# rubengooj/stvo-pl

Hardware: AMD Instinct MI355X
Metric: stereo frames/s (match+optimizePose) (higher is better)
Workload: dtype u8/fp4+f64; 1 GPU; BASELINE configs[2]: KITTI-00-shaped stereo with points + lines (ORB + LBD rows), grid-windowed stereo match (points and lines) + f2f brute-force mutual-NNR match (points and lines) + full GN optimizePose (config_kitti.yaml), device-resident per-frame pipeline; the streams cycle through the 8 sequence ids / 3 KITTI calibrations of configs[4] (sequence s on rank s mod G); streams_per_gpu=3072, parallelism=seq-shard x1

## Files before the change

### stvo-pl_amd/csrc/match_mfma.hip

```cpp
#include <type_traits>

#include "kernels.h"

namespace stvo {

typedef int v4i __attribute__((ext_vector_type(4)));
typedef int v8i __attribute__((ext_vector_type(8)));
typedef int v16i __attribute__((ext_vector_type(16)));
typedef float v16f __attribute__((ext_vector_type(16)));

#ifndef MF_TPB
#define MF_TPB 2
#endif
#ifndef MF_FOLD_SLOTS
#define MF_FOLD_SLOTS 5
#endif
constexpr int MF_BLOCK = 256;
constexpr int MF_TILE = 32;
constexpr int MF_KEY_SHIFT = 13;
constexpr int MF_KEY_BIAS = 1 << 20;
constexpr int MF_NO_KEY = 0x7FFFFFFF;
constexpr int MF_NO_KEY_MIN = 0x40000000;

__device__ __forceinline__ v4i expand_fp4(uint32_t w) {
    v4i r;
    r.x = (int)(((w << 3) & 0x88888888u) | 0x66666666u);
    r.y = (int)(((w << 2) & 0x88888888u) | 0x66666666u);
    r.z = (int)(((w << 1) & 0x88888888u) | 0x66666666u);
    r.w = (int)((w & 0x88888888u) | 0x66666666u);
    return r;
}
__device__ __forceinline__ float med3_f32(float a, float b, float c) {
    float r;
    asm("v_med3_f32 %0, %1, %2, %3" : "=v"(r) : "v"(a), "v"(b), "v"(c));
    return r;
}
__device__ __forceinline__ float min_f32(float a, float b) {
    float r;
    asm("v_min_f32 %0, %1, %2" : "=v"(r) : "v"(a), "v"(b));
    return r;
}
__device__ __forceinline__ float max_f32(float a, float b) {
    float r;
    asm("v_max_f32 %0, %1, %2" : "=v"(r) : "v"(a), "v"(b));
    return r;
}
__device__ __forceinline__ float min3_f32(float a, float b, float c) {
    float r;
    asm("v_min3_f32 %0, %1, %2, %3" : "=v"(r) : "v"(a), "v"(b), "v"(c));
    return r;
}
constexpr float MF_NO_KEY_F = 1.0e30f;
constexpr float MF_NO_KEY_MIN_F = 1.0e29f;
constexpr int MF_SCALE_2_4 = 127 + 4;

__device__ __forceinline__ uint32_t key_to_knn(int key, int base) {
    if (key >= MF_NO_KEY_MIN) return 0xFFFFFFFFu;
    const uint32_t u = (uint32_t)(key + base + MF_KEY_BIAS);
    return ((u >> MF_KEY_SHIFT) << 16) | (u & ((1u << MF_KEY_SHIFT) - 1u));
}

template <int QB, int MODE>
__global__ __launch_bounds__(MF_BLOCK, (QB == 1 ? 4 : QB == 2 ? 3 : 1)) void hamming_knn2_mfma_kernel(int B, int tiles, int ndir, int dir0, int nseg, int row_stride,
                                                                      const uint8_t* __restrict__ d1,
                                                                      const int32_t* __restrict__ n1,
                                                                      const uint8_t* __restrict__ d2,
                                                                      const int32_t* __restrict__ n2,
                                                                      uint2* __restrict__ knn12, uint2* __restrict__ knn21,
                                                                      const int32_t* __restrict__ qsel,
                                                                      const int32_t* __restrict__ nsel,
                                                                      uint32_t* __restrict__ claim_init, int qsel_from_back,
                                                                      const int32_t* __restrict__ tsel,
                                                                      const int32_t* __restrict__ ntsel) {
    constexpr bool GATHER = MODE >= 1, TGATHER = MODE == 2;
    constexpr int ROWS = 4 * QB * 32;
    constexpr int KSTEPS = 4;
    using key_t = float;
    using acc_t = v16f;
    constexpr int NBUF = 2 * MF_TPB;
    __shared__ v4i s_tile[NBUF][KSTEPS * 2 * 32];
    const int per_frame = tiles * ndir * nseg;
    const int L = blockIdx.x;
    const int xcd = L & 7, k = L >> 3;
    int fb = k / per_frame, local = k % per_frame;
    if (MODE == 0 && ndir == 1 && tiles > 1) {
        const int groups = (int)(gridDim.x >> 3) / per_frame;
        const int full_pf = (tiles - 1) * nseg, full = full_pf * groups;
        if (k < full) {
            fb = k / full_pf;
            local = k % full_pf;
        } else {
            fb = (k - full) / nseg;
            local = full_pf + (k - full) % nseg;
        }
    }
    const int b = fb * 8 + xcd;
    if (b >= B) return;
    const int seg = local % nseg;
    const int dir = dir0 + (local / nseg) / tiles;
    const int tile = (local / nseg) % tiles;
    const size_t frame_off = (size_t)b * row_stride;
    const int tid = threadIdx.x, lane = tid & 63, wv = tid >> 6, col = lane & 31, hf = lane >> 5;
    const int q_base = tile * ROWS;
    const uint32_t* __restrict__ Q = reinterpret_cast<const uint32_t*>((dir == 0 ? d1 : d2) + frame_off * STVO_DESC_BYTES);
    uint4 qw[QB][2];
    if (!GATHER) {
#pragma unroll
        for (int qb = 0; qb < QB; ++qb) {
            const int qi = min(q_base + (wv * QB + qb) * 32 + col, row_stride - 1);
            qw[qb][0] = reinterpret_cast<const uint4*>(Q)[2 * qi];
            qw[qb][1] = reinterpret_cast<const uint4*>(Q)[2 * qi + 1];
        }
    }
    const int na = n1[b], nb = n2[b];
    const int nq = GATHER ? nsel[b] : (dir == 0 ? na : nb);
    const int nt_all = TGATHER ? ntsel[b] : (dir == 0 ? nb : na);
    if (TGATHER && nt_all == 0) return;
    const int seg_len = (((nt_all + nseg - 1) / nseg) + MF_TILE - 1) & ~(MF_TILE - 1);
    const int j0 = min(seg * seg_len, nt_all);
    const int nt = min(j0 + seg_len, nt_all);
    if (claim_init && seg == 0 && dir == dir0)
        for (int c = q_base + tid; c < min(q_base + ROWS, row_stride); c += MF_BLOCK) claim_init[frame_off + c] = 0xFFFFFFFFu;
    if (q_base >= nq) return;
    const uint32_t* __restrict__ T = reinterpret_cast<const uint32_t*>((dir == 0 ? d2 : d1) + frame_off * STVO_DESC_BYTES);
    uint2* __restrict__ out = (dir == 0 ? knn12 : knn21) + (size_t)seg * B * row_stride + frame_off;

    const bool wave_active = q_base + wv * QB * 32 < nq;
    v4i qf[QB][KSTEPS];
    auto query_row = [&](int qb) {
        const int q = q_base + (wv * QB + qb) * 32 + col;
        const int qc = q < nq ? q : nq - 1;
        return GATHER ? qsel[frame_off + (qsel_from_back ? row_stride - 1 - qc : qc)] : qc;
    };
    if (GATHER) {
#pragma unroll
        for (int qb = 0; qb < QB; ++qb) {
            const int qi = query_row(qb);
            qw[qb][0] = reinterpret_cast<const uint4*>(Q)[2 * qi];
            qw[qb][1] = reinterpret_cast<const uint4*>(Q)[2 * qi + 1];
        }
    }
#pragma unroll
    for (int qb = 0; qb < QB; ++qb) {
        const uint32_t w[8] = {qw[qb][0].x, qw[qb][0].y, qw[qb][0].z, qw[qb][0].w, qw[qb][1].x, qw[qb][1].y, qw[qb][1].z, qw[qb][1].w};
        const bool up = hf != 0;
        qf[qb][0] = expand_fp4(~(up ? w[1] : w[0]));
        qf[qb][1] = expand_fp4(~(up ? w[3] : w[2]));
        qf[qb][2] = expand_fp4(~(up ? w[5] : w[4]));
        qf[qb][3] = expand_fp4(~(up ? w[7] : w[6]));
    }
    acc_t cidx;
#pragma unroll
    for (int r = 0; r < 16; ++r) cidx[r] = (key_t)((r & 3) + 8 * (r >> 2) + 4 * hf);

    const key_t no_key = MF_NO_KEY_F;
    key_t best[QB], second[QB];
#pragma unroll
    for (int qb = 0; qb < QB; ++qb) best[qb] = second[qb] = no_key;

    const int xr = tid & 31, xk = tid >> 5;
    const int ntiles = (nt - j0 + MF_TILE - 1) / MF_TILE;
    auto fetch = [&](int t) -> uint32_t {
        const int j = j0 + t * MF_TILE + xr;
        if (j >= nt) return 0u;
        const int row = TGATHER ? tsel[frame_off + j] : j;
        return T[(size_t)row * 8 + xk];
    };
    auto stage = [&](int t, uint32_t w) {
        s_tile[t & (NBUF - 1)][xk * 32 + xr] = expand_fp4(w);
    };
#pragma unroll
    for (int i = 0; i < MF_TPB; ++i)
        if (i < ntiles) stage(i, fetch(i));
    __syncthreads();
    auto rebase = [&]() {
#pragma unroll
        for (int qb = 0; qb < QB; ++qb) {
            best[qb] -= (key_t)MF_TILE;
            second[qb] -= (key_t)MF_TILE;
        }
    };
    auto fold = [&](int qb, key_t key) {
        second[qb] = med3_f32(best[qb], second[qb], key);
        best[qb] = min_f32(best[qb], key);
    };
    auto mma = [&](const v4i& tf, const v4i& q, const acc_t& c) -> acc_t {
        const v8i a8 = {tf.x, tf.y, tf.z, tf.w, 0, 0, 0, 0}, b8 = {q.x, q.y, q.z, q.w, 0, 0, 0, 0};
        return __builtin_amdgcn_mfma_scale_f32_32x32x64_f8f6f4(a8, b8, c, 4, 4, 0, MF_SCALE_2_4, 0, MF_SCALE_2_4);
    };
    auto mma_fold = [&](acc_t (&cur)[QB], acc_t (&prev)[QB], int t) {
        if (wave_active) {
            const v4i* frag = s_tile[t & (NBUF - 1)];
            const bool fold_prev = t > 0;
            if (fold_prev) rebase();
            key_t node[QB][5];
            v4i tf = frag[lane];
#pragma unroll
            for (int kk = 0; kk < KSTEPS; ++kk) {
                v4i tf_ahead = tf;
                if (kk < KSTEPS - 1) tf_ahead = frag[(kk + 1) * 64 + lane];
#pragma unroll
                for (int qb = 0; qb < QB; ++qb) cur[qb] = mma(tf, qf[qb][kk], kk == 0 ? cidx : cur[qb]);
                if (fold_prev) {
                    if (QB == 1 && kk == 0) asm volatile("s_nop 7\n\ts_nop 7\n\ts_nop 2" : "+v"(prev[0]));
#pragma unroll
                    for (int qb = 0; qb < QB; ++qb) {
                        const acc_t& p = prev[qb];
                        key_t(&a)[5] = node[qb];
                        if (kk == 0) {
                            a[0] = min3_f32(p[0], p[1], p[2]);
                            a[1] = min3_f32(p[3], p[4], p[5]);
                            second[qb] = min3_f32(second[qb], med3_f32(p[0], p[1], p[2]), med3_f32(p[3], p[4], p[5]));
                        } else if (kk == 1) {
                            a[2] = min3_f32(p[6], p[7], p[8]);
                            a[3] = min3_f32(p[9], p[10], p[11]);
                            second[qb] = min3_f32(second[qb], med3_f32(p[6], p[7], p[8]), med3_f32(p[9], p[10], p[11]));
                        } else if (kk == 2) {
                            a[4] = min3_f32(p[12], p[13], p[14]);
                            const key_t b0 = min3_f32(a[0], a[1], a[2]);
                            second[qb] = min3_f32(second[qb], med3_f32(p[12], p[13], p[14]), med3_f32(a[0], a[1], a[2]));
                            a[0] = b0;
                        } else {
                            const key_t b1 = min3_f32(a[3], a[4], p[15]), n1 = med3_f32(a[3], a[4], p[15]);
                            second[qb] = min3_f32(second[qb], n1, med3_f32(a[0], b1, best[qb]));
                            best[qb] = min3_f32(a[0], b1, best[qb]);
                        }
                    }
                }
                if (kk < KSTEPS - 1) __builtin_amdgcn_sched_group_barrier(0x100, 1, 0);
#pragma unroll
                for (int qb = 0; qb < QB; ++qb) {
                    __builtin_amdgcn_sched_group_barrier(0x008, 1, 0);
                    __builtin_amdgcn_sched_group_barrier(0x002, MF_FOLD_SLOTS, 0);
                }
                tf = tf_ahead;
            }
        }
    };
    acc_t accA[QB], accB[QB];
#pragma unroll
    for (int qb = 0; qb < QB; ++qb)
#pragma unroll
        for (int r = 0; r < 16; ++r) accA[qb][r] = accB[qb][r] = 0;
    static_assert(MF_TPB % 2 == 0, "the accumulator sets alternate tile by tile");
    int t = 0;
    uint32_t w_near[MF_TPB];
#pragma unroll
    for (int i = 0; i < MF_TPB; ++i) {
        w_near[i] = 0;
        if (MF_TPB + i < ntiles) w_near[i] = fetch(MF_TPB + i);
    }
    for (; t + MF_TPB <= ntiles; t += MF_TPB) {
        uint32_t w_far[MF_TPB];
#pragma unroll
        for (int i = 0; i < MF_TPB; ++i) {
            w_far[i] = 0;
            if (t + 2 * MF_TPB + i < ntiles) w_far[i] = fetch(t + 2 * MF_TPB + i);
        }
#pragma unroll
        for (int i = 0; i < MF_TPB; ++i) {
            if ((i & 1) == 0) mma_fold(accA, accB, t + i);
            else mma_fold(accB, accA, t + i);
        }
#pragma unroll
        for (int i = 0; i < MF_TPB; ++i) {
            if (t + MF_TPB + i < ntiles) stage(t + MF_TPB + i, w_near[i]);
            w_near[i] = w_far[i];
        }
        __syncthreads();
    }
#pragma unroll
    for (int i = 0; i < MF_TPB - 1; ++i)
        if (t + i < ntiles) {
            if ((i & 1) == 0) mma_fold(accA, accB, t + i);
            else mma_fold(accB, accA, t + i);
        }
    if (wave_active && ntiles > 0) {
        const int jt = j0 + (ntiles - 1) * MF_TILE;
        const acc_t(&last)[QB] = (ntiles & 1) ? accA : accB;
        rebase();
#pragma unroll
        for (int qb = 0; qb < QB; ++qb)
#pragma unroll
            for (int r = 0; r < 16; ++r) {
                const int jr = jt + (r & 3) + 8 * (r >> 2) + 4 * hf;
                fold(qb, jr < nt ? last[qb][r] : no_key);
            }
    }
    if (!wave_active) return;
#pragma unroll
    for (int qb = 0; qb < QB; ++qb) {
        const int bi = best[qb] >= MF_NO_KEY_MIN_F ? MF_NO_KEY : (int)best[qb];
        const int si = second[qb] >= MF_NO_KEY_MIN_F ? MF_NO_KEY : (int)second[qb];
        const int ob = __shfl_xor(bi, 32), os = __shfl_xor(si, 32);
        const int hi = max(bi, ob);
        const int sec = min(min(si, os), hi);
        const int bst = min(bi, ob);
        const int q = q_base + (wv * QB + qb) * 32 + col;
        const int base = j0 + (ntiles - 1) * MF_TILE;
        if (hf == 0 && q < nq) out[query_row(qb)] = make_uint2(key_to_knn(bst, base), key_to_knn(sec, base));
    }
}

constexpr int REV_CHUNK_TILES = 8, REV_CHUNK = REV_CHUNK_TILES * MF_TILE;

__global__ __launch_bounds__(MF_BLOCK, 4) void hamming_knn2_mfma_reverse_kernel(int B, int slots, int row_stride, const uint8_t* __restrict__ d1,
                                                                                const int32_t* __restrict__ n1, const uint8_t* __restrict__ d2,
                                                                                const int32_t* __restrict__ qsel, const int32_t* __restrict__ nsel,
                                                                                const int32_t* __restrict__ tsel, const uint32_t* __restrict__ claim,
                                                                                float nnr, int32_t* __restrict__ m12) {
    constexpr int KSTEPS = 4;
    using key_t = float;
    using acc_t = v16f;
    __shared__ v4i s_tile[REV_CHUNK_TILES][KSTEPS * 2 * 32];
    __shared__ uint16_t s_thr[257];
    const int L = blockIdx.x;
    const int xcd = L & 7, k = L >> 3;
    const int b = (k / slots) * 8 + xcd, slot = k % slots;
    if (b >= B) return;
    const int na = n1[b];
    const int nl = nsel[(size_t)B + b], nh = nsel[2 * (size_t)B + b], ns = nsel[3 * (size_t)B + b];
    if ((ns == 0 || nl == 0) && nh == 0) return;
    {
        const float f0 = (float)threadIdx.x;
        uint32_t thr = threadIdx.x;
        while (thr < 256u && !(f0 < (float)(thr + 1u) * nnr)) ++thr;
        s_thr[threadIdx.x] = (uint16_t)thr;
        if (threadIdx.x == 0) s_thr[256] = 256;
    }
    const size_t frame_off = (size_t)b * row_stride;
    const int tid = threadIdx.x, lane = tid & 63, wv = tid >> 6, col = lane & 31, hf = lane >> 5;
    const int xr = tid & 31, xk = tid >> 5;
    const uint32_t* __restrict__ Q = reinterpret_cast<const uint32_t*>(d2 + frame_off * STVO_DESC_BYTES);
    const uint32_t* __restrict__ T = reinterpret_cast<const uint32_t*>(d1 + frame_off * STVO_DESC_BYTES);
    acc_t cidx;
#pragma unroll
    for (int r = 0; r < 16; ++r) cidx[r] = (key_t)((r & 3) + 8 * (r >> 2) + 4 * hf);
    auto mma = [&](const v4i& tf, const v4i& q, const acc_t& c) -> acc_t {
        const v8i a8 = {tf.x, tf.y, tf.z, tf.w, 0, 0, 0, 0}, b8 = {q.x, q.y, q.z, q.w, 0, 0, 0, 0};
        return __builtin_amdgcn_mfma_scale_f32_32x32x64_f8f6f4(a8, b8, c, 4, 4, 0, MF_SCALE_2_4, 0, MF_SCALE_2_4);
    };

    for (int list = 0; list < 2; ++list) {
        const bool light = list == 0;
        const int nq = light ? (ns > 0 ? nl : 0) : nh, nt_all = light ? ns : na;
        if (nq == 0) continue;
        const int nseg = rev_segments(nt_all);
        const int n_groups = (nq + 127) / 128;
        const int seg_len = (((nt_all + nseg - 1) / nseg) + MF_TILE - 1) & ~(MF_TILE - 1);
        auto column_of = [&](int g) -> int {
            const int q = (g * 4 + wv) * 32 + col;
            return q < nq ? q : nq - 1;
        };
        auto list_entry = [&](int g) -> int { return qsel[frame_off + (light ? column_of(g) : row_stride - 1 - column_of(g))]; };
        for (int seg = 0; seg < nseg; ++seg) {
            const int g_first = ((slot - seg) % slots + slots) % slots;
            if (g_first >= n_groups) continue;
            const int j0 = min(seg * seg_len, nt_all), nt = min(j0 + seg_len, nt_all);
            for (int c0 = j0; c0 < nt || c0 == j0; c0 += REV_CHUNK) {
                uint32_t w[REV_CHUNK_TILES];
#pragma unroll
                for (int t = 0; t < REV_CHUNK_TILES; ++t) {
                    const int j = c0 + t * MF_TILE + xr;
                    uint32_t v = 0u;
                    if (j < nt) v = T[(size_t)(light ? tsel[frame_off + j] : j) * 8 + xk];
                    w[t] = v;
                }
                int e_cur = list_entry(g_first);
                int e_next = g_first + slots < n_groups ? list_entry(g_first + slots) : 0;
                const int ntc = min((nt - c0 + MF_TILE - 1) / MF_TILE, REV_CHUNK_TILES);
#pragma unroll
                for (int t = 0; t < REV_CHUNK_TILES; ++t)
                    if (t < ntc) s_tile[t][xk * 32 + xr] = expand_fp4(w[t]);
                uint4 qw0 = reinterpret_cast<const uint4*>(Q)[2 * e_cur], qw1 = reinterpret_cast<const uint4*>(Q)[2 * e_cur + 1];
                uint32_t cw = claim[frame_off + e_cur];
                __syncthreads();
                for (int g = g_first; g < n_groups; g += slots) {
                    const bool up = hf != 0;
                    v4i qf[KSTEPS];
                    qf[0] = expand_fp4(~(up ? qw0.y : qw0.x));
                    qf[1] = expand_fp4(~(up ? qw0.w : qw0.z));
                    qf[2] = expand_fp4(~(up ? qw1.y : qw1.x));
                    qf[3] = expand_fp4(~(up ? qw1.w : qw1.z));
                    const uint32_t c_claim = cw;
                    const bool block_active = (g * 4 + wv) * 32 < nq;
                    if (g + slots < n_groups) {
                        qw0 = reinterpret_cast<const uint4*>(Q)[2 * e_next];
                        qw1 = reinterpret_cast<const uint4*>(Q)[2 * e_next + 1];
                        cw = claim[frame_off + e_next];
                        e_cur = e_next;
                        if (g + 2 * slots < n_groups) e_next = list_entry(g + 2 * slots);
                    }
                    if (!block_active) continue;
                    key_t best = MF_NO_KEY_F, second = MF_NO_KEY_F;
                    auto fold = [&](key_t key) {
                        second = med3_f32(best, second, key);
                        best = min_f32(best, key);
                    };
                    int last_base = c0;
                    if (ntc > 0) {
                        auto do_tile = [&](acc_t& cur, acc_t& prev, int t) {
                            key_t nd[5];
                            const v4i* frag = s_tile[t];
                            const bool fold_prev = t > 0;
                            if (fold_prev) {
                                best -= (key_t)MF_TILE;
                                second -= (key_t)MF_TILE;
                            }
                            v4i tf = frag[lane];
#pragma unroll
                            for (int kk = 0; kk < KSTEPS; ++kk) {
                                v4i tf_ahead = tf;
                                if (kk < KSTEPS - 1) tf_ahead = frag[(kk + 1) * 64 + lane];
                                cur = mma(tf, qf[kk], kk == 0 ? cidx : cur);
                                if (fold_prev) {
                                    if (kk == 0) {
                                        asm volatile("s_nop 7\n\ts_nop 7\n\ts_nop 2" : "+v"(prev));
                                        nd[0] = min3_f32(prev[0], prev[1], prev[2]);
                                        nd[1] = min3_f32(prev[3], prev[4], prev[5]);
                                        second = min3_f32(second, med3_f32(prev[0], prev[1], prev[2]), med3_f32(prev[3], prev[4], prev[5]));
                                    } else if (kk == 1) {
                                        nd[2] = min3_f32(prev[6], prev[7], prev[8]);
                                        nd[3] = min3_f32(prev[9], prev[10], prev[11]);
                                        second = min3_f32(second, med3_f32(prev[6], prev[7], prev[8]), med3_f32(prev[9], prev[10], prev[11]));
                                    } else if (kk == 2) {
                                        nd[4] = min3_f32(prev[12], prev[13], prev[14]);
                                        const key_t b0 = min3_f32(nd[0], nd[1], nd[2]);
                                        second = min3_f32(second, med3_f32(prev[12], prev[13], prev[14]), med3_f32(nd[0], nd[1], nd[2]));
                                        nd[0] = b0;
                                    } else {
                                        const key_t b1 = min3_f32(nd[3], nd[4], prev[15]), n1 = med3_f32(nd[3], nd[4], prev[15]);
                                        second = min3_f32(second, n1, med3_f32(nd[0], b1, best));
                                        best = min3_f32(nd[0], b1, best);
                                    }
                                }
                                if (kk < KSTEPS - 1) __builtin_amdgcn_sched_group_barrier(0x100, 1, 0);
                                __builtin_amdgcn_sched_group_barrier(0x008, 1, 0);
                                __builtin_amdgcn_sched_group_barrier(0x002, MF_FOLD_SLOTS, 0);
                                tf = tf_ahead;
                            }
                        };
                        acc_t accA, accB;
#pragma unroll
                        for (int r = 0; r < 16; ++r) accA[r] = accB[r] = 0;
                        int t = 0;
                        for (; t + 2 <= ntc; t += 2) {
                            do_tile(accA, accB, t);
                            do_tile(accB, accA, t + 1);
                        }
                        if (t < ntc) do_tile(accA, accB, t);
                        acc_t& last = (ntc & 1) ? accA : accB;
                        asm volatile("s_nop 7\n\ts_nop 7\n\ts_nop 2" : "+v"(last));
                        best -= (key_t)MF_TILE;
                        second -= (key_t)MF_TILE;
                        last_base = c0 + (ntc - 1) * MF_TILE;
#pragma unroll
                        for (int r = 0; r < 16; ++r) {
                            const int jr = last_base + (r & 3) + 8 * (r >> 2) + 4 * hf;
                            fold(jr < nt ? last[r] : MF_NO_KEY_F);
                        }
                    }
                    const int bi = best >= MF_NO_KEY_MIN_F ? MF_NO_KEY : (int)best;
                    const int si = second >= MF_NO_KEY_MIN_F ? MF_NO_KEY : (int)second;
                    const int ob = __shfl_xor(bi, 32), os = __shfl_xor(si, 32);
                    const int hi = max(bi, ob);
                    const int sec = min(min(si, os), hi);
                    const int bst = min(bi, ob);
                    if (hf == 0 && (g * 4 + wv) * 32 + col < nq) {
                        const uint32_t x = key_to_knn(bst, last_base), y = key_to_knn(sec, last_base);
                        if (x != 0xFFFFFFFFu) {
                            const uint32_t T = s_thr[c_claim >> 16], istar = c_claim & 0xFFFFu;
                            bool blk = false;
                            if ((x >> 16) <= T) {
                                const uint32_t pos = x & 0xFFFFu;
                                const uint32_t row = light ? (uint32_t)tsel[frame_off + pos] : pos;
                                blk = row != istar || (y != 0xFFFFFFFFu && (y >> 16) <= T);
                            }
                            if (blk) m12[frame_off + istar] = -1;
                        }
                    }
                }
                __syncthreads();
            }
        }
    }
}

void launch_hamming_knn2_mfma_reverse(hipStream_t s, int B, int row_stride, const uint8_t* d1, const int32_t* n1, const uint8_t* d2, const int32_t* qsel,
                                      const int32_t* nsel, const int32_t* tsel, const uint32_t* claim, float nnr, int32_t* m12, int slots) {
    if (B <= 0 || row_stride <= 0) return;
    const dim3 grid((unsigned)(((B + 7) / 8) * 8 * slots));
    hipLaunchKernelGGL(hamming_knn2_mfma_reverse_kernel, grid, dim3(MF_BLOCK), 0, s, B, slots, row_stride, d1, n1, d2, qsel, nsel, tsel, claim, nnr, m12);
}

int mfma_rows_per_block(int qb) { return 4 * qb * 32; }

template <int QB, int MODE>
static void launch_mf(dim3 grid, hipStream_t s, int B, int tiles, int ndir, int dir0, int nseg, int row_stride, const uint8_t* d1,
                      const int32_t* n1, const uint8_t* d2, const int32_t* n2, uint2* knn12, uint2* knn21, const int32_t* qsel,
                      const int32_t* nsel, uint32_t* claim_init, int qsel_from_back, const int32_t* tsel, const int32_t* ntsel) {
    hipLaunchKernelGGL((hamming_knn2_mfma_kernel<QB, MODE>), grid, dim3(MF_BLOCK), 0, s, B, tiles, ndir, dir0, nseg, row_stride, d1, n1, d2, n2,
                       knn12, knn21, qsel, nsel, claim_init, qsel_from_back, tsel, ntsel);
}

void launch_hamming_knn2_mfma(hipStream_t s, int B, int row_stride, int max_n, const uint8_t* d1, const int32_t* n1,
                              const uint8_t* d2, const int32_t* n2, uint2* knn12, uint2* knn21, int both_directions,
                              int dir0, const int32_t* qsel, const int32_t* nsel, int nseg, uint32_t* claim_init, int qb,
                              int qsel_from_back, const int32_t* tsel, const int32_t* ntsel) {
    if (B <= 0 || max_n <= 0) return;
    const int rows = mfma_rows_per_block(qb);
    const int tiles = (max_n + rows - 1) / rows, ndir = both_directions ? 2 : 1;
    const int groups = (B + 7) / 8;
    const dim3 grid((unsigned)(groups * 8 * tiles * ndir * nseg));
#define STVO_MF_ARGS grid, s, B, tiles, ndir, dir0, nseg, row_stride, d1, n1, d2, n2, knn12, knn21, qsel, nsel, claim_init, qsel_from_back, tsel, ntsel
    if (qsel || tsel) return;
    if (qb == 1) launch_mf<1, 0>(STVO_MF_ARGS);
    else if (qb == 2) launch_mf<2, 0>(STVO_MF_ARGS);
    else launch_mf<4, 0>(STVO_MF_ARGS);
#undef STVO_MF_ARGS
}

}
```

Baseline: 1.367 million frame-pairs/s.

## Use ±6 fp4 encoding, paired-tile rebase, clamped fetches in forward MFMA kNN

After: 1.402 million frame-pairs/s (median of 6 runs). +2.6%, better.

```diff
diff --git a/stvo-pl_amd/csrc/match_mfma.hip b/stvo-pl_amd/csrc/match_mfma.hip
--- a/stvo-pl_amd/csrc/match_mfma.hip
+++ b/stvo-pl_amd/csrc/match_mfma.hip
@@ -15,10 +15,21 @@
 #ifndef MF_FOLD_SLOTS
 #define MF_FOLD_SLOTS 5
 #endif
+#ifndef MF_PM6
+#define MF_PM6 1
+#endif
+#ifndef MF_PAIR_REBASE
+#define MF_PAIR_REBASE 1
+#endif
+#ifndef MF_CLAMP_FETCH
+#define MF_CLAMP_FETCH 1
+#endif
 constexpr int MF_BLOCK = 256;
 constexpr int MF_TILE = 32;
 constexpr int MF_KEY_SHIFT = 13;
 constexpr int MF_KEY_BIAS = 1 << 20;
+constexpr int MF_FWD_UNIT = MF_PM6 ? 18432 : 1 << MF_KEY_SHIFT;
+constexpr int MF_FWD_BIAS = MF_PM6 ? 256 * 9216 : MF_KEY_BIAS;
 constexpr int MF_NO_KEY = 0x7FFFFFFF;
 constexpr int MF_NO_KEY_MIN = 0x40000000;
 
@@ -30,6 +41,16 @@
     r.w = (int)((w & 0x88888888u) | 0x66666666u);
     return r;
 }
+__device__ __forceinline__ v4i expand_fp4_pm6(uint32_t w) {
+    v4i r;
+    r.x = (int)((w << 3) | 0x77777777u);
+    r.y = (int)((w << 2) | 0x77777777u);
+    r.z = (int)((w << 1) | 0x77777777u);
+    r.w = (int)(w | 0x77777777u);
+    return r;
+}
+__device__ __forceinline__ v4i expand_fwd(uint32_t w) { return MF_PM6 ? expand_fp4_pm6(w) : expand_fp4(w); }
+typedef float v2f __attribute__((ext_vector_type(2)));
 __device__ __forceinline__ float med3_f32(float a, float b, float c) {
     float r;
     asm("v_med3_f32 %0, %1, %2, %3" : "=v"(r) : "v"(a), "v"(b), "v"(c));
@@ -58,6 +79,13 @@
     if (key >= MF_NO_KEY_MIN) return 0xFFFFFFFFu;
     const uint32_t u = (uint32_t)(key + base + MF_KEY_BIAS);
     return ((u >> MF_KEY_SHIFT) << 16) | (u & ((1u << MF_KEY_SHIFT) - 1u));
+}
+
+__device__ __forceinline__ uint32_t key_to_knn_fwd(int key, int base) {
+    if (key >= MF_NO_KEY_MIN) return 0xFFFFFFFFu;
+    const uint32_t u = (uint32_t)(key + base + MF_FWD_BIAS);
+    const uint32_t h = u / (uint32_t)MF_FWD_UNIT;
+    return (h << 16) | (u - h * (uint32_t)MF_FWD_UNIT);
 }
 
 template <int QB, int MODE>
@@ -144,14 +172,19 @@
     for (int qb = 0; qb < QB; ++qb) {
         const uint32_t w[8] = {qw[qb][0].x, qw[qb][0].y, qw[qb][0].z, qw[qb][0].w, qw[qb][1].x, qw[qb][1].y, qw[qb][1].z, qw[qb][1].w};
         const bool up = hf != 0;
-        qf[qb][0] = expand_fp4(~(up ? w[1] : w[0]));
-        qf[qb][1] = expand_fp4(~(up ? w[3] : w[2]));
-        qf[qb][2] = expand_fp4(~(up ? w[5] : w[4]));
-        qf[qb][3] = expand_fp4(~(up ? w[7] : w[6]));
-    }
-    acc_t cidx;
-#pragma unroll
-    for (int r = 0; r < 16; ++r) cidx[r] = (key_t)((r & 3) + 8 * (r >> 2) + 4 * hf);
+        qf[qb][0] = expand_fwd(~(up ? w[1] : w[0]));
+        qf[qb][1] = expand_fwd(~(up ? w[3] : w[2]));
+        qf[qb][2] = expand_fwd(~(up ? w[5] : w[4]));
+        qf[qb][3] = expand_fwd(~(up ? w[7] : w[6]));
+    }
+    constexpr bool PAIR = MF_PAIR_REBASE != 0 && QB <= 2;
+    constexpr int REBASE = PAIR ? 2 * MF_TILE : MF_TILE;
+    acc_t cidx, cidx_odd;
+#pragma unroll
+    for (int r = 0; r < 16; ++r) {
+        cidx[r] = (key_t)((r & 3) + 8 * (r >> 2) + 4 * hf);
+        cidx_odd[r] = cidx[r] + (key_t)(PAIR ? MF_TILE : 0);
+    }
 
     const key_t no_key = MF_NO_KEY_F;
     key_t best[QB], second[QB];
@@ -160,24 +193,41 @@
 
     const int xr = tid & 31, xk = tid >> 5;
     const int ntiles = (nt - j0 + MF_TILE - 1) / MF_TILE;
+    constexpr bool CLAMPED = MF_CLAMP_FETCH != 0 && !TGATHER;
+    const int slot_last = (row_stride - 1) * STVO_DESC_BYTES;
+    const uint32_t lane_off = (uint32_t)(xr * STVO_DESC_BYTES + xk * 4);
     auto fetch = [&](int t) -> uint32_t {
-        const int j = j0 + t * MF_TILE + xr;
-        if (j >= nt) return 0u;
-        const int row = TGATHER ? tsel[frame_off + j] : j;
-        return T[(size_t)row * 8 + xk];
+        if constexpr (CLAMPED) {
+            const int tile_off = min((j0 + t * MF_TILE) * STVO_DESC_BYTES, slot_last);
+            const uint32_t off = min(lane_off, (uint32_t)(slot_last - tile_off + STVO_DESC_BYTES - 4));
+            return *reinterpret_cast<const uint32_t*>(reinterpret_cast<const char*>(T) + (size_t)tile_off + (size_t)off);
+        } else {
+            const int j = j0 + t * MF_TILE + xr;
+            if (j >= nt) return 0u;
+            const int row = TGATHER ? tsel[frame_off + j] : j;
+            return T[(size_t)row * 8 + xk];
+        }
     };
     auto stage = [&](int t, uint32_t w) {
-        s_tile[t & (NBUF - 1)][xk * 32 + xr] = expand_fp4(w);
+        s_tile[t & (NBUF - 1)][xk * 32 + xr] = expand_fwd(w);
     };
 #pragma unroll
     for (int i = 0; i < MF_TPB; ++i)
         if (i < ntiles) stage(i, fetch(i));
     __syncthreads();
+    const v2f rebase2 = {-(key_t)REBASE, -(key_t)REBASE};
     auto rebase = [&]() {
 #pragma unroll
         for (int qb = 0; qb < QB; ++qb) {
-            best[qb] -= (key_t)MF_TILE;
-            second[qb] -= (key_t)MF_TILE;
+            if constexpr (PAIR) {
+                v2f bs = {best[qb], second[qb]};
+                asm("v_pk_add_f32 %0, %0, %1" : "+v"(bs) : "s"(rebase2));
+                best[qb] = bs.x;
+                second[qb] = bs.y;
+            } else {
+                best[qb] -= (key_t)MF_TILE;
+                second[qb] -= (key_t)MF_TILE;
+            }
         }
     };
     auto fold = [&](int qb, key_t key) {
@@ -192,7 +242,8 @@
         if (wave_active) {
             const v4i* frag = s_tile[t & (NBUF - 1)];
             const bool fold_prev = t > 0;
-            if (fold_prev) rebase();
+            const bool odd = (t & 1) != 0;
+            if (fold_prev && (!PAIR || odd)) rebase();
             key_t node[QB][5];
             v4i tf = frag[lane];
 #pragma unroll
@@ -200,7 +251,7 @@
                 v4i tf_ahead = tf;
                 if (kk < KSTEPS - 1) tf_ahead = frag[(kk + 1) * 64 + lane];
 #pragma unroll
-                for (int qb = 0; qb < QB; ++qb) cur[qb] = mma(tf, qf[qb][kk], kk == 0 ? cidx : cur[qb]);
+                for (int qb = 0; qb < QB; ++qb) cur[qb] = mma(tf, qf[qb][kk], kk == 0 ? (odd ? cidx_odd : cidx) : cur[qb]);
                 if (fold_prev) {
                     if (QB == 1 && kk == 0) asm volatile("s_nop 7\n\ts_nop 7\n\ts_nop 2" : "+v"(prev[0]));
 #pragma unroll
@@ -226,6 +277,9 @@
                             best[qb] = min3_f32(a[0], b1, best[qb]);
                         }
                     }
+                } else if (kk == KSTEPS - 1 && ntiles > 1) {
+#pragma unroll
+                    for (int qb = 0; qb < QB; ++qb) asm volatile("s_nop 7\n\ts_nop 7" : "+v"(cur[qb]));
                 }
                 if (kk < KSTEPS - 1) __builtin_amdgcn_sched_group_barrier(0x100, 1, 0);
 #pragma unroll
@@ -235,6 +289,7 @@
                 }
                 tf = tf_ahead;
             }
+            __builtin_amdgcn_sched_barrier(0);
         }
     };
     acc_t accA[QB], accB[QB];
@@ -244,18 +299,17 @@
         for (int r = 0; r < 16; ++r) accA[qb][r] = accB[qb][r] = 0;
     static_assert(MF_TPB % 2 == 0, "the accumulator sets alternate tile by tile");
     int t = 0;
-    uint32_t w_near[MF_TPB];
+    uint32_t w_near[MF_TPB], w_far[MF_TPB];
 #pragma unroll
     for (int i = 0; i < MF_TPB; ++i) {
-        w_near[i] = 0;
-        if (MF_TPB + i < ntiles) w_near[i] = fetch(MF_TPB + i);
-    }
-    for (; t + MF_TPB <= ntiles; t += MF_TPB) {
-        uint32_t w_far[MF_TPB];
+        w_near[i] = w_far[i] = 0;
+        if (CLAMPED || MF_TPB + i < ntiles) w_near[i] = fetch(MF_TPB + i);
+    }
+    auto trip = [&](uint32_t (&w_stage)[MF_TPB], uint32_t (&w_fetch)[MF_TPB]) {
 #pragma unroll
         for (int i = 0; i < MF_TPB; ++i) {
-            w_far[i] = 0;
-            if (t + 2 * MF_TPB + i < ntiles) w_far[i] = fetch(t + 2 * MF_TPB + i);
+            if (!CLAMPED) w_fetch[i] = 0;
+            if (CLAMPED || t + 2 * MF_TPB + i < ntiles) w_fetch[i] = fetch(t + 2 * MF_TPB + i);
         }
 #pragma unroll
         for (int i = 0; i < MF_TPB; ++i) {
@@ -263,11 +317,23 @@
             else mma_fold(accB, accA, t + i);
         }
 #pragma unroll
-        for (int i = 0; i < MF_TPB; ++i) {
-            if (t + MF_TPB + i < ntiles) stage(t + MF_TPB + i, w_near[i]);
-            w_near[i] = w_far[i];
-        }
+        for (int i = 0; i < MF_TPB; ++i)
+            if (t + MF_TPB + i < ntiles) stage(t + MF_TPB + i, w_stage[i]);
         __syncthreads();
+        t += MF_TPB;
+    };
+    if (CLAMPED) {
+        while (t + MF_TPB <= ntiles) {
+            trip(w_near, w_far);
+            if (t + MF_TPB > ntiles) break;
+            trip(w_far, w_near);
+        }
+    } else {
+        while (t + MF_TPB <= ntiles) {
+            trip(w_near, w_far);
+#pragma unroll
+            for (int i = 0; i < MF_TPB; ++i) w_near[i] = w_far[i];
+        }
     }
 #pragma unroll
     for (int i = 0; i < MF_TPB - 1; ++i)
@@ -278,7 +344,7 @@
     if (wave_active && ntiles > 0) {
         const int jt = j0 + (ntiles - 1) * MF_TILE;
         const acc_t(&last)[QB] = (ntiles & 1) ? accA : accB;
-        rebase();
+        if (!PAIR || (ntiles & 1)) rebase();
 #pragma unroll
         for (int qb = 0; qb < QB; ++qb)
 #pragma unroll
@@ -297,8 +363,8 @@
         const int sec = min(min(si, os), hi);
         const int bst = min(bi, ob);
         const int q = q_base + (wv * QB + qb) * 32 + col;
-        const int base = j0 + (ntiles - 1) * MF_TILE;
-        if (hf == 0 && q < nq) out[query_row(qb)] = make_uint2(key_to_knn(bst, base), key_to_knn(sec, base));
+        const int base = j0 + (PAIR ? (ntiles - 1) & ~1 : ntiles - 1) * MF_TILE;
+        if (hf == 0 && q < nq) out[query_row(qb)] = make_uint2(key_to_knn_fwd(bst, base), key_to_knn_fwd(sec, base));
     }
 }
 
```
